# IntelRealSense/hand_tracking_samples

Measured on AMD Instinct MI355X. Metric: synthetic depth frames/sec (CNN+solver), 64x64x1 input, 17-bone hand, higher is better.
Workload: dtype f32; 1 GPU; BASELINE configs[2]: 1024 independent 64x64 frames per GPU, CNN + decode + 5-step MultiStepSim + 3 FitPointCloud passes (GJK + PGS), 17 bones; frames_per_gpu=1024, parallelism=single GPU

## Files before the change

### hand_tracking_samples_amd/csrc/ht_gjk.hip

```cpp
#include <stdlib.h>
#include <mutex>
#include "ht_device.hpp"
#include "ht_launch.hpp"

extern __shared__ __attribute__((aligned(16))) float4 g_sm[];

typedef float f32x2 __attribute__((ext_vector_type(2)));
struct support_t { int voff, n; v3 pos; v4 q; int outer; v3 opos; v4 oq; int sub, grp; };
struct mkpoint { v3 a, b; float t; __device__ __forceinline__ v3 p() const { return a - b; } };
struct simplex { v3 v; mkpoint W[4]; int count; };
struct gjk_hit { v3 normal, p0w, p1w; float separation; };

__device__ __forceinline__ v3 support_inner(const support_t &s, v3 dir)
{
	const v3 dl = qrot(qconj(s.q), dir);
	const float4 *vs = g_sm + s.voff;
	float4 q0 = vs[0];
	float best = dot(V3(q0.x, q0.y, q0.z), dl); int bi = 0;
	const f32x2 dlxy = { dl.x, dl.y };
	int i = 6 * s.sub;
	for (; i + 6 <= s.n; i += 6 * s.grp)
	{
		const float4 *g = vs + i;
		float d[6]; int id[6];
// ... 1056 lines not shown
		}
	}
}

size_t ht_contacts_workspace_bytes(int B) { (void)B; return 16; }

int ht_contacts_frames_per_block(const ht_model_dev &M, int B)
{
	const size_t fixed = (size_t)M.cvert_off[M.nb] * sizeof(float4) + sizeof(co_block) + (size_t)CO_OWN * 64 * 2 * (sizeof(co_req) + sizeof(int)) + CO_EPAQ * sizeof(co_job) + CO_NW * gjk_wave_stride();
	if (fixed + sizeof(co_frame) > 160 * 1024) return 0;
	int nfr = CO_MAXF;
	while (nfr > 1 && fixed + nfr * sizeof(co_frame) > 160 * 1024) nfr--;
	return B < nfr ? B : nfr;
}
#define CO_ORDER_SEG 4096
__global__ __launch_bounds__(1024) void k_contact_order(const int *__restrict__ work, int *__restrict__ order, int Ball, int nfr, int stride, unsigned slots, int epb)
{
	extern __shared__ int ko_w[];
	__shared__ int ko_ne;
	if (!((slots >> blockIdx.x) & 1u)) return;
	const int seg = (CO_ORDER_SEG / nfr) * nfr, f0 = blockIdx.y * seg, B = Ball - f0 < seg ? Ball - f0 : seg;
	const int blocks_all = (Ball + nfr - 1) / nfr, b0 = f0 / nfr;
	const int *w = work + (size_t)blockIdx.x * stride + f0;
	int *o = order + (size_t)blockIdx.x * stride;
	const int blocks = (B + nfr - 1) / nfr, B4 = (B + 3) & ~3;
	if (threadIdx.x == 0) ko_ne = 0;
	__syncthreads();
	int mine = 0;
	for (int i = threadIdx.x; i < B4; i += 1024)
	{
		const int v = i < B ? w[i] : -1;
		const int runs = v < 0 ? 0 : (v >> 16), pairs = v < 0 ? 0 : (v & 0xffff);
		ko_w[i] = v < 0 ? -1 : ((runs > 1023 ? 1023 : runs) << 20) | pairs;
		mine += runs > 0 ? 1 : 0;
	}
	if (mine) atomicAdd(&ko_ne, mine);
	for (int i = threadIdx.x; i < blocks * nfr; i += 1024) o[(i / blocks) * blocks_all + b0 + i % blocks] = Ball;
	__syncthreads();
	const int ne = ko_ne, ng = B - ne;
	if (epb > nfr) epb = nfr;
	if (epb * blocks < ne) epb = (ne + blocks - 1) / blocks;
	const int neb = (ne + epb - 1) / epb, ngb = blocks - neb;
	const int nfree = neb * nfr - ne;
	const int nheavy = ng - nfree > 0 ? ng - nfree : 0;
	for (int i = threadIdx.x; i < B; i += 1024)
	{
		const int wi = ko_w[i];
		int rank = 0;
		for (int j = 0; j < B4; j += 4)
		{
			const int4 k = *reinterpret_cast<const int4 *>(ko_w + j);
			rank += ((k.x > wi || (k.x == wi && j < i)) ? 1 : 0) + ((k.y > wi || (k.y == wi && j + 1 < i)) ? 1 : 0) + ((k.z > wi || (k.z == wi && j + 2 < i)) ? 1 : 0) + ((k.w > wi || (k.w == wi && j + 3 < i)) ? 1 : 0);
		}
		int nb_, base, r;
		if (rank < ne) { nb_ = neb; base = 0; r = rank; }
		else if (rank - ne < nheavy) { nb_ = ngb; base = neb; r = rank - ne; }
		else { nb_ = neb; base = 0; r = ne + (rank - ne - nheavy); }
		const int round = r / nb_, pos = r - round * nb_;
		o[round * blocks_all + b0 + base + ((round & 1) ? nb_ - 1 - pos : pos)] = f0 + i;
	}
}
void ht_launch_contact_order(const int *work, int *order, int B, int nfr, int stride, unsigned slots, int nslots, int epb, hipStream_t s)
{
	const int seg = (CO_ORDER_SEG / nfr) * nfr, nseg = (B + seg - 1) / seg;
	hipLaunchKernelGGL(k_contact_order, dim3(nslots, nseg), dim3(1024), (size_t)(((B < seg ? B : seg) + 3) & ~3) * sizeof(int), s, work, order, B, nfr, stride, slots, epb);
}
void ht_launch_contacts(const ht_model_dev &M, const float *state, float driftmax, float jiggle_sin, const int *active_flag, void *epa_ws, float *contacts, int *ncontacts, int B, hipStream_t s, bool beside_cloud_rows, int force_kernel, int few_frames,
                        const int *order, int *work_out)
{
	int *caps = reinterpret_cast<int *>(epa_ws);
	const int dbg = ht_tuning_flags();
	static bool attr_set[64];
	static std::mutex attr_lock;
	int dev = 0; (void)hipGetDevice(&dev); dev &= 63;
	std::unique_lock<std::mutex> lk(attr_lock);
	if (!attr_set[dev])
	{
		(void)hipFuncSetAttribute(reinterpret_cast<const void *>(k_contacts<1>), hipFuncAttributeMaxDynamicSharedMemorySize, 160 * 1024);
		(void)hipFuncSetAttribute(reinterpret_cast<const void *>(k_contacts<2>), hipFuncAttributeMaxDynamicSharedMemorySize, 160 * 1024);
		(void)hipFuncSetAttribute(reinterpret_cast<const void *>(k_contacts_coop), hipFuncAttributeMaxDynamicSharedMemorySize, 160 * 1024);
// ... 30 lines not shown
```

### hand_tracking_samples_amd/csrc/ht_host.hpp

```cpp
#pragma once
#include <map>
#include <string>
#include <vector>
#include "ht_device.hpp"

struct ht_comm_state;
struct ht_prof_entry { std::vector<hipEvent_t> ev; size_t used; float total_ms; int launches; };

struct ht_ctx
{
	bool ready = false, have_weights = false, profile = false;
	bool cnn_only = false;
	bool profile_phases = false;
	int B = 0, device = 0;
	int solver_build = 0;
	float *d_exact_lin = nullptr, *d_exact_ang = nullptr;
	int contact_kernel = 0;
	std::string err;
	hipStream_t stream = nullptr;
	hipStream_t last_user_stream = nullptr;
	hipStream_t side[2] = { nullptr, nullptr };
	hipEvent_t ev_fork = nullptr, ev_join[2] = { nullptr, nullptr }, ev_lap = nullptr;
	unsigned side_open = 0;
	hipEvent_t ev_job = nullptr, ev_seed = nullptr; bool job_pending = false; void *h_job_in = nullptr; size_t h_job_cap = 0;
// ... 22 lines not shown
	float *d_state[2] = { nullptr, nullptr };
	float *d_prev_err = nullptr; int *d_initializing = nullptr;
	float *d_err_old = nullptr, *d_err_new = nullptr; int *d_flags = nullptr, *d_nflags = nullptr;
	int *d_flist = nullptr, *d_nflist = nullptr;
	unsigned *d_nreset = nullptr; volatile unsigned *h_nreset = nullptr;
	unsigned nreset_seen[2] = { 0, 0 }; bool many_reset = false, tail_pending = false; int n_cu = 256;
	int last_reset_many = -1;
	float *d_rows = nullptr; int *d_nrows = nullptr;
	unsigned char *d_rowbody = nullptr;
	float *d_chamber = nullptr; int *d_nchamber = nullptr;
	float *d_tables = nullptr;
	float *d_chplanes = nullptr; int *d_chon = nullptr; bool planes_valid = false;
	int solve_tables = 0;
	int *d_accepted = nullptr;
	float *d_contacts = nullptr; int *d_ncontacts = nullptr;
	int *d_cwork = nullptr, *d_corder = nullptr;
	int *d_porder = nullptr;
	int *d_swork = nullptr, *d_sorder = nullptr; unsigned swork_mask = 0, sorder_mask = 0; int swork_B = 0;
	int cstride = 0, cwork_B = 0; unsigned cwork_mask = 0, corder_mask = 0;
	unsigned char *d_epa_ws = nullptr;
	float *d_scratch = nullptr;
	float *d_poses_out = nullptr, *d_start = nullptr;
	float *d_stage = nullptr;
	float *d_user_lin = nullptr; unsigned short *d_user_pos = nullptr; float *d_user_ang = nullptr; int *d_user_n = nullptr;
	int user_lin_cap = 0, user_ang_cap = 0;
	ht_comm_state *comm = nullptr;
	char *d_render = nullptr; size_t render_cap = 0;
	char *d_labels = nullptr; size_t labels_cap = 0;
	char *d_segment = nullptr; size_t segment_cap = 0;
	std::vector<float4> render_planes; std::vector<float> render_radii;
// ... 69 lines not shown
```

### hand_tracking_samples_amd/csrc/ht_solver.hip

```cpp
#include "ht_solve_shared.hpp"

template <int NGRP_, int NSUM_, int NANG_, int NIDX_, int AS_ = 2, int NCG_ = 0> struct lds_t
{
	static constexpr int NGRP = NGRP_, NSUM = NSUM_, NANG = NANG_, NIDX = NIDX_, MAXA2 = MAXA2_OF(AS_), NCG = NCG_;
	static constexpr int LIDLE = MAXG - 1;
	float pool[NGRP * LGRP] __attribute__((aligned(16)));
	float4 lin4[HT_MAXNB];
	float4 ang4[HT_MAXNB];
	float pos[HT_MAXNB][3], q[HT_MAXNB][4];
	float csum[NSUM];
	unsigned short cidx[NIDX > 0 ? NIDX : 2];
	float cg[NCG];
	int ccnt[HT_MAXNB], cstart[HT_MAXNB];
	signed char cextra[HT_MAXNB];
	union
	{
		unsigned lorder[MAXG];
		struct { unsigned short abody[128]; unsigned etmp[64]; } blk;
	};
	unsigned short lstart[MAXG + 2];
	unsigned aorder[MAXA2 + 1];
	unsigned short astart[MAXA2 + 2];
	int nlev_lin, nlev_ang, nray;
	union
// ... 1360 lines not shown
		if (bad) { pos = L3(bc + HT_BC_POS0); q = L4(bc + HT_BC_Q0); lin = V3(0, 0, 0); ang = V3(0, 0, 0); }
		if (a.zero_momenta) { lin = V3(0, 0, 0); ang = V3(0, 0, 0); }
		s[0] = pos.x; s[1] = pos.y; s[2] = pos.z; s[3] = q.x; s[4] = q.y; s[5] = q.z; s[6] = q.w;
		s[7] = lin.x; s[8] = lin.y; s[9] = lin.z; s[10] = ang.x; s[11] = ang.y; s[12] = ang.z;
		if (a.out_poses)
		{
			const v3 pu = apply(XF(pos, q), -L3(bc + HT_BC_COM));
			float *o = a.out_poses + ((size_t)b * nb + lane) * HT_POSE;
			o[0] = pu.x; o[1] = pu.y; o[2] = pu.z; o[3] = q.x; o[4] = q.y; o[5] = q.z; o[6] = q.w;
			if (lane == 0 && a.out_npts[b] < a.out_min_point_num) a.out_initializing[b] = 50;
		}
	}
	if (a.cost_out && lane == 0) a.cost_out[b] = (int)((clock64() - t_cost) >> 4);
}

__global__ __launch_bounds__(1024) void k_rank_desc(const int *__restrict__ work, int *__restrict__ order, int Ball, int stride, unsigned slots)
{
	__shared__ int rk_w[4096];
	if (!((slots >> blockIdx.x) & 1u)) return;
	const int f0 = blockIdx.y * 4096, B = Ball - f0 < 4096 ? Ball - f0 : 4096, B4 = (B + 3) & ~3;
	const int *w = work + (size_t)blockIdx.x * stride + f0;
	int *o = order + (size_t)blockIdx.x * stride + f0;
	for (int i = threadIdx.x; i < B4; i += 1024) rk_w[i] = i < B ? w[i] : -1;
	__syncthreads();
	for (int i = threadIdx.x; i < B; i += 1024)
	{
		const int wi = rk_w[i];
		int rank = 0;
		for (int j = 0; j < B4; j += 4)
		{
			const int4 k = *reinterpret_cast<const int4 *>(rk_w + j);
			rank += ((k.x > wi || (k.x == wi && j < i)) ? 1 : 0) + ((k.y > wi || (k.y == wi && j + 1 < i)) ? 1 : 0) + ((k.z > wi || (k.z == wi && j + 2 < i)) ? 1 : 0) + ((k.w > wi || (k.w == wi && j + 3 < i)) ? 1 : 0);
		}
		o[rank] = f0 + i;
	}
}
void ht_launch_rank_desc(const int *work, int *order, int B, int stride, unsigned slots, int nslots, hipStream_t s)
{
	hipLaunchKernelGGL(k_rank_desc, dim3(nslots, (B + 4095) / 4096), dim3(1024), 0, s, work, order, B, stride, slots);
}

#define SOLVE_ONLY_NCG 1440
static_assert(sizeof(lds_t<66, 1024, 126, 1024, 2, SOLVE_ONLY_NCG>) <= 40960, "the build for 1024 frames must fit four times into a CU's LDS");
static_assert(sizeof(lds_t<34, 584, 84, 0>) <= 20480, "the small build must leave room for eight frames per CU (160 KB of LDS)");
static_assert(HT_SCRATCH_TAIL * HT_CREC >= MAXG_CAP * LGRP + (MAXA_CAP_OF(4) + 4) * AROW + HT_CREC, "the tail of a frame's scratch slot must hold its linear groups, its angular records and the tuning record");
void ht_launch_solve(const ht_model_dev &M, const ht_physics_dev &ph, const solve_args &a, int B, hipStream_t s)
{
	const int pts = M.pts_bound > 0 ? M.pts_bound : M.pts_cap;
	const bool tile = M.nj + 8 + 1 <= 38 && pts <= 1024;
	int build = a.force_build;
	if (build == 7) { solve_args b = a; b.force_build = 0; b.two_body_levels = 1; ht_launch_solve(M, ph, b, B, s); return; }
	if (!build) build = tile ? (B <= 1024 && !a.shared_gpu ? 2 : 1) : 3;
	if (build >= 1 && build <= 3 && 13 + 6 * M.nj + a.ang_extra_bound > MAXA_CAP_OF(2)) build = 6;
	if (build == 2) hipLaunchKernelGGL((k_solve<66, 1024, 126, 1024, false, 2, SOLVE_ONLY_NCG>), dim3(B), dim3(64), 0, s, M, ph, a);
// ... 7 lines not shown
```

### hand_tracking_samples_amd/csrc/ht_solver_api.hip

```cpp
#include <string.h>
#include <stdlib.h>
#include "ht_device.hpp"
#include "ht_host.hpp"
#include "ht_launch.hpp"

#define CHECK_RANGE(ctx, first, n) do { if ((first) < 0 || (n) < 1 || (first) + (n) > (ctx)->B) { (ctx)->err = "slot range exceeds the capacity given to ht_create"; return HT_ERR_ARG; } } while (0)

static int scratch_stride(const ht_ctx *ctx) { return (int)ht_scratch_rows((size_t)ctx->model.pts_cap, (size_t)ctx->model.nb); }

static int dev_alloc_points(ht_ctx *ctx)
{
	const int r = dev_alloc(ctx, &ctx->d_ptsv, (size_t)ctx->B * ctx->model.pts_cap);
	return r || ctx->d_nptsv ? r : dev_alloc(ctx, &ctx->d_nptsv, (size_t)ctx->B);
}
static cloud_records cloud_rec(ht_ctx *ctx) { cloud_records r = { ctx->d_scratch, scratch_stride(ctx), ctx->d_rowbody, ctx->phys.deltaT }; return r; }
static bool exact_solver(const ht_ctx *ctx) { return ctx->solver_build == 5 || ctx->solver_build == 8; }
static const cloud_records *rec_or_rows(const ht_ctx *ctx, const cloud_records *cr) { return exact_solver(ctx) ? nullptr : cr; }
static void exact_args(ht_ctx *ctx, solve_args &a, bool cloud)
{
	a.force_build = exact_solver(ctx) ? 5 : ctx->solver_build;
	a.exact_lin = ctx->d_exact_lin; a.exact_ang = ctx->d_exact_ang;
	if (exact_solver(ctx) && cloud) { a.rows_cloud = ctx->d_rows; a.cloud_body = nullptr; }
}
#define REFUSE_EXACT_SOLVER(ctx) do { if (exact_solver(ctx)) { (ctx)->err = "the exact-order instantiation (ht_debug_solver_build 5) serves the update entry points only"; return HT_ERR_STATE; } } while (0)
// ... 4 lines not shown
	a.analysis = ctx->d_analysis; a.cams = ctx->d_cams; a.state = ctx->d_state[which]; a.scratch = ctx->d_scratch; a.scratch_stride = scratch_stride(ctx); a.batch = ctx->B;
	return a;
}
struct step_mix { bool angles, rays, cloud, chamber; float palm_drive; int arm_cone, zero_momenta; };
static step_mix mix_of_step(const ht_params &p, int st)
{
	const bool angles = (st < p.steps_keyangles) || p.angles_only, rays = (st < p.steps_keypoints) && !p.angles_only, cloud = (st >= p.steps_cloudstart) && !p.angles_only;
	step_mix m = { angles, rays, cloud, false, st < p.steps_palmangle ? 10000.0f : 0.0f, 1, 1 };
	return m;
}
static step_mix mix_of_pass() { step_mix m = { false, false, true, true, 0.0f, 0, 0 }; return m; }
static int step_slot(int st) { return st < 8 ? st : -1; }
static int pass_slot(int pass) { return pass >= 0 && pass < 8 ? 8 + pass : -1; }
static bool solve_history_on(const ht_ctx *ctx, int B) { return ctx->d_swork && B > ctx->n_cu * 8 && B + 8 <= ctx->cstride; }
struct solve_opts { const int *active = nullptr; int hist_slot = -1; bool tables = false, shared_gpu = false; float *poses_out = nullptr; const int *out_npts = nullptr; };
static void solve_step(ht_ctx *ctx, int which, const step_mix &m, int B, hipStream_t s, const solve_opts &o)
{
	solve_args a = solve_head(ctx, which, ctx->phys.use_collision != 0);
	a.rows_pre = m.chamber ? ctx->d_chamber : nullptr; a.n_pre = m.chamber ? ctx->d_nchamber : nullptr; a.pre_stride = 5 * ctx->model.nb;
	a.cloud_body = m.cloud ? ctx->d_rowbody : nullptr; a.n_cloud = ctx->d_nrows;
	a.active_flag = o.active; a.apply_angles = m.angles; a.drive_force = m.palm_drive; a.ray_rows = m.rays; a.arm_cone = m.arm_cone; a.zero_momenta = m.zero_momenta;
	a.steps_keyangles = ctx->par.steps_keyangles; a.min_cray_prob = ctx->par.min_cray_prob;
	a.dbg = ht_tuning_flags(); a.shared_gpu = o.shared_gpu ? 1 : 0; a.tables = o.tables ? ctx->d_tables : nullptr;
	exact_args(ctx, a, m.cloud);
	a.out_poses = o.poses_out; a.out_npts = o.out_npts; a.out_initializing = ctx->d_initializing; a.out_min_point_num = ctx->par.min_point_num;
	if (o.hist_slot >= 0 && o.hist_slot < HT_CONTACT_SLOTS && !o.active && !exact_solver(ctx) && solve_history_on(ctx, B) && B == ctx->swork_B)
	{
		a.cost_out = ctx->d_swork + (size_t)o.hist_slot * ctx->cstride;
		ctx->swork_mask |= 1u << o.hist_slot;
		if ((ctx->sorder_mask >> o.hist_slot) & 1u) a.frame_order = ctx->d_sorder + (size_t)o.hist_slot * ctx->cstride;
	}
	ht_launch_solve(ctx->model, ctx->phys, a, B, s);
}
static int solve_tables_mode(const ht_ctx *ctx)
{
	static const int env = ht_tuning_int("HT_TABLES", -1);
	const int m = env >= 0 ? env : ctx->solve_tables;
	return (m && ctx->d_tables && !exact_solver(ctx)) ? m : 0;
}
static bool solve_tables_on(const ht_ctx *ctx) { return solve_tables_mode(ctx) == 1; }
static void solve_prep(ht_ctx *ctx, int which, const step_mix &m, bool pose_only, const int *active, int B, hipStream_t s)
{
	prep_args a;
	memset(&a, 0, sizeof a);
	a.state = ctx->d_state[which]; a.analysis = ctx->d_analysis; a.cams = ctx->d_cams; a.active_flag = active;
	a.scratch = ctx->d_scratch; a.scratch_stride = scratch_stride(ctx); a.batch = ctx->B;
// ... 21 lines not shown
static inline void marks_dump() {}
#endif
struct contact_slot { const int *order; int *work; };
static contact_slot contact_history(ht_ctx *ctx, int slot, const int *active, int B)
{
	contact_slot c = { nullptr, nullptr };
	if (slot < 0 || slot >= HT_CONTACT_SLOTS || !ctx->d_cwork || active == ctx->d_flags || B != ctx->cwork_B) return c;
	c.work = ctx->d_cwork + (size_t)slot * ctx->cstride;
	ctx->cwork_mask |= 1u << slot;
	if ((ctx->corder_mask >> slot) & 1u) c.order = ctx->d_corder + (size_t)slot * ctx->cstride;
	return c;
}
static void launch_contacts(ht_ctx *ctx, int which, const int *active, int B, hipStream_t s, bool beside_cloud_rows = false, int slot = -1)
{
	const contact_slot ch = contact_history(ctx, slot, active, B);
	ht_launch_contacts(ctx->model, ctx->d_state[which], ctx->phys.driftmax, ctx->phys.jiggle_sin, active, ctx->d_epa_ws, ctx->d_contacts, ctx->d_ncontacts, B, s, beside_cloud_rows, ctx->contact_kernel,
	                   active && active == ctx->d_flags && !ctx->many_reset, ch.order, ch.work);
}
static void contact_orders(ht_ctx *ctx, int B, hipStream_t t)
{
	const int nfr = ht_contacts_frames_per_block(ctx->model, B);
	ctx->corder_mask = 0;
	if (ctx->d_cwork && ctx->cwork_B == B && ctx->cwork_mask && nfr > 1 && B + 8 <= ctx->cstride && ctx->contact_kernel != 2)
	{
		static const int epb_env = ht_tuning_int("HT_CONTACT_EPB", 0);
		const int blocks = (B + nfr - 1) / nfr;
		ht_launch_contact_order(ctx->d_cwork, ctx->d_corder, B, nfr, ctx->cstride, ctx->cwork_mask, HT_CONTACT_SLOTS, epb_env > 0 ? epb_env : blocks > ctx->n_cu ? nfr : 1, t);
		ctx->corder_mask = ctx->cwork_mask;
	}
	ctx->cwork_mask = 0; ctx->cwork_B = B;
	ctx->sorder_mask = 0;
	if (solve_history_on(ctx, B) && ctx->swork_B == B && ctx->swork_mask)
	{
		ht_launch_rank_desc(ctx->d_swork, ctx->d_sorder, B, ctx->cstride, ctx->swork_mask, HT_CONTACT_SLOTS, t);
		ctx->sorder_mask = ctx->swork_mask;
	}
	ctx->swork_mask = 0; ctx->swork_B = B;
}
static void fork(ht_ctx *ctx, hipStream_t s) { (void)hipEventRecord(ctx->ev_fork, s); for (int i = 0; i < 2; i++) (void)hipStreamWaitEvent(ctx->side[i], ctx->ev_fork, 0); ctx->side_open |= 3u; }
static void fork1(ht_ctx *ctx, hipStream_t s, int i) { (void)hipEventRecord(ctx->ev_fork, s); (void)hipStreamWaitEvent(ctx->side[i], ctx->ev_fork, 0); ctx->side_open |= 1u << i; }
static void join1(ht_ctx *ctx, hipStream_t s, int i) { (void)hipEventRecord(ctx->ev_join[i], ctx->side[i]); (void)hipStreamWaitEvent(s, ctx->ev_join[i], 0); ctx->side_open &= ~(1u << i); }
static void join(ht_ctx *ctx, hipStream_t s, int n) { for (int i = 0; i < n; i++) join1(ctx, s, i); }
static void join_open(ht_ctx *ctx, hipStream_t s) { for (int i = 0; i < 2; i++) if ((ctx->side_open >> i) & 1u) join1(ctx, s, i); }

struct steps_on
{
	hipStream_t s; int from = 0, to = 1 << 30; const int *active = nullptr; int side = 0; bool prof = true, shared_gpu = false, rows = true, solve = true;
	explicit steps_on(hipStream_t stream) : s(stream) {}
	steps_on &steps(int first, int end = 1 << 30) { from = first; to = end; return *this; }
	steps_on &frames(const int *flags) { active = flags; return *this; }
	steps_on &all_frames() { active = nullptr; return *this; }
	steps_on &rows_beside(int i) { side = i; return *this; }
	steps_on &in_order() { side = -1; return *this; }
	steps_on &unprofiled() { prof = false; return *this; }
	steps_on &shares_gpu() { shared_gpu = true; return *this; }
	steps_on &rows_only() { solve = false; return *this; }
// ... 123 lines not shown
static void update_planes(ht_ctx *ctx, const update_call &u, hipStream_t t)
{
	const ht_params &p = ctx->par;
	if (u.mode == UPD_CNN_MODEL || u.mode == UPD_KICKSTART || p.angles_only || p.mainthreadpasses < 1) return;
	ht_launch_chamber_planes(ctx->model, p.subsample_voxel ? ctx->d_ptsv : ctx->d_pts, p.subsample_voxel ? ctx->d_nptsv : ctx->d_npts, p.min_point_num, p.boundary_planes, ctx->d_chplanes, ctx->d_chon, u.B, t); ctx->planes_valid = true;
}
static void update_fit_error_old(ht_ctx *ctx, const update_call &u, hipStream_t t)
{
	const ht_params &p = ctx->par;
	ht_fit_after dec; memset(&dec, 0, sizeof dec);
	dec.mode = 1; dec.reset_thr = p.full_reset_on_error; dec.angles_only = p.angles_only; dec.flags = ctx->d_flags; dec.nflags = ctx->d_nflags; dec.list = ctx->d_flist; dec.nlist = ctx->d_nflist; dec.nreset = ctx->d_nreset;
	ht_launch_fit_error(ctx->model, ctx->d_state[0], ctx->d_pts, ctx->d_npts, u.d_depth, u.img_cams, u.iw, u.ih, p.bone_sum_error_scale, ctx->d_err_old, u.B, t, &dec);
}
static void update_beside_net(ht_ctx *ctx, const update_call &u)
{
	hipStream_t t = ctx->side[1];
	fork(ctx, u.s);
	update_planes(ctx, u, t);
	contact_orders(ctx, u.B, t);
	if (u.mode == UPD_FULL && !(u.d_start && !u.fs)) ht_launch_set_pose(ctx->d_state[1], ctx->d_state[0], ctx->model.nb, u.B, 2, t);
	update_fit_error_old(ctx, u, t);
}
static void update_net(ht_ctx *ctx, const update_call &u, bool overlap)
{
	const frame_src *fs = u.fs; const bool direct = fs && fs->direct; hipStream_t s = u.s;
	ht_prof_scope ps(ctx, direct ? "cnn128" : "cnn", s, true);
	if (direct) ht_launch_cnn(ctx->cnnw128, ctx->d_in128, ctx->d_act1_128, ctx->d_act2_128, ctx->d_act3, ctx->d_logits, u.B, s, fs->direct, overlap);
	else ht_launch_cnn(ctx->cnnw, ctx->d_cnn_in, ctx->d_act1, ctx->d_act2, ctx->d_act3, ctx->d_logits, u.B, s, 64, overlap);
	ht_launch_softmax_decode(ctx->d_logits, u.d_cnn_out ? u.d_cnn_out : ctx->d_cnn_out, ctx->d_cams, ctx->d_analysis, 1, u.B, s, direct ? fs->direct / 16 : 4);
}
static void resets_short(ht_ctx *ctx, int B, hipStream_t s)
{
	reset_path(ctx, true, ctx->par.steps_unibody, B, ctx->side[0], s, ctx->many_reset);
	multistep(ctx, B, steps_on(s).steps(0, 1).frames(ctx->d_nflags).rows_beside(0).shares_gpu());
	join(ctx, s, 1); reset_tail(ctx);
	multistep(ctx, B, steps_on(s).steps(0, 1).frames(ctx->d_flags).rows_beside(0));
// ... 7 lines not shown
	join(ctx, s, 1); reset_tail(ctx);
	multistep(ctx, B, steps_on(s).steps(join_step).all_frames().rows_beside(0));
}
static void resets_lap(ht_ctx *ctx, int B, hipStream_t s)
{
	hipStream_t u = ctx->side[0];
	const int *reset_frames = ctx->d_flags, *batch_frames = ctx->d_nflags;
	mark("fork", s);
	reset_path(ctx, true, ctx->par.steps_unibody, B, s, s, ctx->many_reset); mark("reset kernel done", s);
	multistep(ctx, B, steps_on(u).steps(0, 1).frames(batch_frames).in_order().unprofiled().shares_gpu()); mark("batch step 0 done", u);
	multistep(ctx, B, steps_on(s).steps(0, 1).frames(reset_frames).in_order().rows_only()); mark("reset frames contacts done", s);
	(void)hipEventRecord(ctx->ev_lap, s); (void)hipStreamWaitEvent(u, ctx->ev_lap, 0);
	multistep(ctx, B, steps_on(s).steps(0, 1).frames(reset_frames).in_order().solve_only()); mark("reset frames step 0 done", s);
	multistep(ctx, B, steps_on(u).steps(1, 2).frames(batch_frames).in_order().unprofiled().rows_only()); mark("batch step 1 rows done", u);
	multistep(ctx, B, steps_on(s).steps(1, 2).frames(reset_frames).rows_beside(1).rows_only()); mark("reset frames step 1 rows done", s);
	join(ctx, s, 1); reset_tail(ctx);
	multistep(ctx, B, steps_on(s).steps(1, 2).all_frames().solve_only()); mark("step 1 done", s);
	multistep(ctx, B, steps_on(s).steps(2).all_frames().rows_beside(0)); mark("MultiStepSim done", s);
}
static void update_resets(ht_ctx *ctx, const update_call &u)
{
	hipStream_t s = u.s; join1(ctx, s, 1);
	static const int join_step = ht_tuning_int("HT_RESET_JOIN", 0);
	fork(ctx, s);
	const unsigned frames = ctx->h_nreset[0], updates = ctx->h_nreset[1];
	if (updates != ctx->nreset_seen[1])
	{
		ctx->many_reset = (frames - ctx->nreset_seen[0]) / (updates - ctx->nreset_seen[1]) > (unsigned)ctx->n_cu;
		ctx->nreset_seen[0] = frames; ctx->nreset_seen[1] = updates;
	}
	static const bool no_lap = ht_tuning_env("HT_NO_STEP1_LAP");
	if (join_step > 0) resets_joined_late(ctx, u.B, s, join_step);
	else if (ctx->par.steps >= 2 && !no_lap) resets_lap(ctx, u.B, s);
	else resets_short(ctx, u.B, s);
}
static void update_accept(ht_ctx *ctx, const update_call &u)
{
	const ht_params &p = ctx->par;
	ht_fit_after acc; memset(&acc, 0, sizeof acc);
	acc.mode = 2; acc.hand = u.mode == UPD_CNN_MODEL ? nullptr : ctx->d_state[0]; acc.other = ctx->d_state[1]; acc.err_old = ctx->d_err_old; acc.prev_err = ctx->d_prev_err;
	acc.initializing = ctx->d_initializing; acc.accepted = ctx->d_accepted; acc.nb = ctx->model.nb; acc.min_point_num = p.min_point_num; acc.always_take_cnn = p.always_take_cnn;
	acc.angles_only = p.angles_only; acc.accum_thr = p.accum_error_threshold; ht_prof_scope ps(ctx, "fit_error", u.s, true);
	ht_launch_fit_error(ctx->model, ctx->d_state[1], ctx->d_pts, ctx->d_npts, u.d_depth, u.img_cams, u.iw, u.ih, p.bone_sum_error_scale, ctx->d_err_new, u.B, u.s, &acc);
}
static void update_passes(ht_ctx *ctx, const update_call &u)
{
	const ht_params &p = ctx->par;
	const int passes = p.angles_only ? 0 : p.mainthreadpasses;
// ... 434 lines not shown
}
extern "C" int ht_debug_reset_flags(ht_ctx *ctx, int *flags, int n)
{
	if (!ctx || !flags || n < 0 || n > ctx->B) return HT_ERR_ARG;
	ht_device_guard dev_guard_(ctx->device);
	HIPCHK(ctx, hipStreamSynchronize(ctx->stream));
	HIPCHK(ctx, hipMemcpy(flags, ctx->d_flags, (size_t)n * sizeof(int), hipMemcpyDeviceToHost));
	return HT_OK;
}
extern "C" int ht_debug_contact_kernel(ht_ctx *ctx, int which)
{
	if (!ctx || which < 0 || which > 2) return HT_ERR_ARG;
	ctx->contact_kernel = which;
	return HT_OK;
}
extern "C" int ht_debug_solve_tables(ht_ctx *ctx, int on)
{
	if (!ctx || !ctx->ready) return HT_ERR_ARG;
	ht_device_guard dev_guard_(ctx->device);
	if (on < 0 || on > 2) return HT_ERR_ARG;
	if (on) { const int r = ht_alloc_solve_tables(ctx); if (r) return r; }
	ctx->solve_tables = on;
	return HT_OK;
}
extern "C" int ht_debug_solve_tables_header(ht_ctx *ctx, int B, int *hdr)
{
	if (!ctx || !ctx->ready || !hdr || B < 1 || B > ctx->B || !ctx->d_tables) return HT_ERR_ARG;
	ht_device_guard dev_guard_(ctx->device);
	if (ht_sync_all(ctx) != hipSuccess) return HT_ERR_HIP;
	if (hipMemcpy2D(hdr, 32 * sizeof(int), ctx->d_tables, (size_t)TB_WORDS * sizeof(float), 32 * sizeof(int), B, hipMemcpyDeviceToHost) != hipSuccess) return HT_ERR_HIP;
// ... 233 lines not shown
```

### hand_tracking_samples_amd/native.py

```python
import ctypes as C
import os

import numpy as np

from . import build as _build

HERE = os.path.dirname(os.path.abspath(__file__))
HT_OK = 0
CNN_IN, CNN_OUT, CNNB_COUNT, POSE, STATE, CAM, ANALYSIS = 4096, 2304, 9458400, 7, 13, 12, 84
MAXPTS, ROW, CONTACT = 4096, 16, 12
LABELS_SEGMENT_FRAME = 1
TRAIN_ACT = (("a1", 57600, (16, 60, 60)), ("a3", 3600, (16, 15, 15)), ("a5", 9216, (64, 12, 12)), ("a6", 2304, (2304,)), ("a8", 2048, (2048,)))
TRAIN_ERR = (("e9", 2304, (2304,)), ("e7", 2048, (2048,)), ("e6", 2304, (2304,)), ("part3", 57600, (16, 3600)), ("sqp", 9, (9,)), (None, 7, None))

SYMBOLS = (
    "ht_create", "ht_destroy", "ht_model_bake", "ht_last_error", "ht_get_params", "ht_set_params", "ht_model_info", "ht_config_read", "ht_scale",
    "ht_cnn_load_weights", "ht_cnn_eval", "ht_cnn_eval_dev", "ht_cnn_load_weights_sized", "ht_cnn_eval_sized", "ht_cnn_eval_sized_dev", "ht_cnn_train", "ht_cnn_get_weights", "ht_expected_cnn", "ht_expected_cnn_full",
    "ht_expected_cnn_batch", "ht_expected_cnn_dev", "ht_cnn_input_dev", "ht_cnn_train_dev", "ht_cnn_train_batch_dev", "ht_cnn_train_batch", "ht_debug_train_batch_buffers",
    "ht_model_open", "ht_model_close", "ht_model_error", "ht_model_counts", "ht_model_body", "ht_model_body_mesh", "ht_model_body_sdmesh", "ht_model_hitcheck", "ht_model_hitcheck_mesh", "ht_model_render_mesh", "ht_model_scale", "ht_render_mesh_depth", "ht_render_mesh_depth_dev",
    "ht_tracker_reset", "ht_get_state", "ht_set_state", "ht_get_tracker_flags", "ht_set_tracker_flags", "ht_update_sync", "ht_update_dev", "ht_update_frames_sync", "ht_update_frames_dev", "ht_update_direct_sync", "ht_update_direct_dev", "ht_update_cnn_model_sync", "ht_get_cnn_results", "ht_get_cnn_layers", "ht_frames_overflow", "ht_reserve_points", "ht_point_capacity", "ht_capacity_events", "ht_segment_vr", "ht_segment_vr_dev", "ht_render_depth", "ht_render_depth_dev", "ht_slowfit", "ht_set_points", "ht_fit_rows", "ht_physics_update",
    "ht_stage_prepare", "ht_stage_decode", "ht_stage_fit_error", "ht_stage_cloud_rows", "ht_stage_contacts", "ht_stage_fit",
    "ht_stage_multistep", "ht_stage_multistep_range", "ht_stage_scratch_unibody", "ht_stage_chamber", "ht_profile_enable", "ht_profile_read", "ht_debug_solve_stats", "ht_debug_contact_stats", "ht_debug_solver_build", "ht_debug_reset_flags", "ht_debug_reset_organisation", "ht_update_passes_sync", "ht_job_start", "ht_job_poll", "ht_job_wait", "ht_job_collect", "ht_debug_contact_kernel", "ht_contact_capacity", "ht_debug_solve_tables", "ht_debug_solve_tables_header", "ht_debug_train_buffers",
    "ht_comm_available", "ht_comm_unique_id", "ht_comm_init", "ht_comm_info", "ht_gather_poses_dev", "ht_gather_wait", "ht_gather_wait_host", "ht_comm_destroy",
)


class Params(C.Structure):
    _fields_ = [("full_reset_on_error", C.c_float), ("angles_only", C.c_int), ("always_take_cnn", C.c_int), ("drangey", C.c_float), ("boundary_planes", C.c_int),
                ("microforce", C.c_float), ("cloudforce_max_point", C.c_float), ("cloudforce_max_sum", C.c_float), ("mainthreadpasses", C.c_int),
                ("subsample_fraction", C.c_int), ("min_point_num", C.c_int), ("accum_error_threshold", C.c_float), ("min_cray_prob", C.c_float),
                ("steps", C.c_int), ("steps_keypoints", C.c_int), ("steps_keyangles", C.c_int), ("steps_palmangle", C.c_int), ("steps_cloudstart", C.c_int), ("steps_unibody", C.c_int),
                ("physics_iterations", C.c_int), ("physics_iterations_post", C.c_int), ("physics_use_collision", C.c_int),
                ("physics_weak_force", C.c_float), ("bone_sum_error_scale", C.c_float), ("unibody_force", C.c_float),
                ("subsample_voxel", C.c_int), ("subsample_size", C.c_float)]


class HTError(RuntimeError):
# ... 76 lines not shown
    L.ht_segment_vr.argtypes = [vp, C.POINTER(C.c_uint16), fp, C.c_int, C.c_int, C.c_int, C.c_int, C.c_float, C.c_float, C.c_float, C.POINTER(C.c_uint16), fp]
    L.ht_segment_vr_dev.argtypes = [vp, vp, vp, C.c_int, C.c_int, C.c_int, C.c_int, C.c_float, C.c_float, C.c_float, vp, vp, vp]
    L.ht_render_depth.argtypes = [vp, fp, fp, C.c_int, C.c_int, C.c_float, C.c_int, u16p, C.POINTER(C.c_int8)]
    L.ht_render_depth_dev.argtypes = [vp, vp, vp, C.c_int, C.c_int, C.c_float, C.c_int, vp, vp, vp]
    L.ht_render_mesh_depth.argtypes = [vp, fp, fp, C.c_int, C.c_int, C.c_float, C.c_float, C.c_int, u16p, C.POINTER(C.c_int8)]
    L.ht_render_mesh_depth_dev.argtypes = [vp, vp, vp, C.c_int, C.c_int, C.c_float, C.c_float, C.c_int, vp, vp, vp]
    L.ht_model_hitcheck_mesh.argtypes = [vp, fp, fp, fp, fp, fp, ip, ip]
    L.ht_model_render_mesh.argtypes = [vp, fp, fp, C.c_int, C.c_int, C.c_float, C.c_float, u16p, C.POINTER(C.c_int8)]
    L.ht_model_scale.argtypes = [vp, C.c_float]
    L.ht_profile_read.argtypes = [vp, C.c_int, C.c_int, C.c_char_p, C.c_int, fp, ip, ip]
    L.ht_debug_solve_stats.argtypes = [vp, C.c_int, fp, C.c_int]
    L.ht_debug_solver_build.argtypes = [vp, C.c_int]
    L.ht_debug_reset_organisation.argtypes = [vp, ip]
    L.ht_debug_reset_flags.argtypes = [vp, ip, C.c_int]
    L.ht_debug_contact_kernel.argtypes = [vp, C.c_int]
    L.ht_debug_solve_tables.argtypes = [vp, C.c_int]
    L.ht_contact_capacity.argtypes = [vp, ip, ip, ip, ip]
    L.ht_debug_solve_tables_header.argtypes = [vp, C.c_int, ip]
    L.ht_comm_unique_id.argtypes = [vp]
    L.ht_comm_init.argtypes = [vp, C.c_int, C.c_int, vp]
    L.ht_comm_info.argtypes = [vp, ip, ip]
    L.ht_gather_poses_dev.argtypes = [vp, vp, vp, C.c_int, C.c_int, vp]
    L.ht_gather_wait.argtypes = [vp, C.c_int, vp]
    L.ht_gather_wait_host.argtypes = [vp, C.c_int]
    L.ht_comm_available.argtypes = []
    L.ht_comm_destroy.argtypes = [vp]
    L.ht_debug_contact_stats.argtypes = [vp, C.c_int, fp, C.c_int]
    for name in SYMBOLS:
        if name not in ("ht_last_error", "ht_model_error"):
            getattr(L, name).restype = C.c_int
# ... 302 lines not shown

    def gather_wait_host(self, slot):
        self._chk(self.L.ht_gather_wait_host(self.h, int(slot)))

    def debug_reset_flags(self, n):
        f = np.zeros(n, np.int32)
        self._chk(self.L.ht_debug_reset_flags(self.h, f.ctypes.data_as(C.POINTER(C.c_int)), n))
        return f

    def debug_solver_build(self, which):
        self._chk(self.L.ht_debug_solver_build(self.h, int(which)))

    def debug_contact_kernel(self, which):
        self._chk(self.L.ht_debug_contact_kernel(self.h, int(which)))

    def contact_capacity(self):
        v = [C.c_int() for _ in range(4)]
        self._chk(self.L.ht_contact_capacity(self.h, *[C.byref(x) for x in v]))
        return tuple(x.value for x in v)

    def debug_solve_tables(self, on):
        self._chk(self.L.ht_debug_solve_tables(self.h, int(on)))

    def debug_solve_tables_header(self, B):
        h = np.zeros((B, 32), np.int32)
        self._chk(self.L.ht_debug_solve_tables_header(self.h, B, _i(h)))
        return h

    def debug_contact_stats(self, B, reset=True):
        out = np.zeros((B, 24), np.float32)
# ... 175 lines not shown
```

### include/ht_mi355x.h

```cpp
#ifndef HT_MI355X_H
#define HT_MI355X_H
#include <stddef.h>
#include <stdint.h>

#ifdef __cplusplus
extern "C" {
#endif

#define HT_OK 0
#define HT_ERR_ARG 1
#define HT_ERR_IO 2
#define HT_ERR_HIP 3
#define HT_ERR_STATE 4

#define HT_CNN_IN 4096
#define HT_CNN_OUT 2304
#define HT_CNNB_COUNT 9458400
#define HT_CNN128_IN 16384
#define HT_CNNB128_COUNT 30429920
#define HT_POSE 7
#define HT_STATE 13
#define HT_CAM 12
#define HT_MAX_POINTS 4096
#define HT_POINTS_LIMIT 76800
// ... 130 lines not shown
int ht_comm_unique_id(void *id128);
int ht_comm_init(ht_ctx *ctx, int world, int rank, const void *id128);
int ht_comm_info(ht_ctx *ctx, int *world, int *rank);
int ht_gather_poses_dev(ht_ctx *ctx, const float *d_local, float *d_all, int frames, int slot, void *stream);
int ht_gather_wait(ht_ctx *ctx, int slot, void *stream);
int ht_comm_destroy(ht_ctx *ctx);

int ht_profile_enable(ht_ctx *ctx, int on);
int ht_profile_read(ht_ctx *ctx, int reset, int max_entries, char *names, int name_stride, float *total_ms, int *launches, int *n_entries);
int ht_debug_solve_stats(ht_ctx *ctx, int B, float *out, int reset);
int ht_debug_contact_stats(ht_ctx *ctx, int B, float *out, int reset);
int ht_debug_solver_build(ht_ctx *ctx, int which);
int ht_debug_reset_flags(ht_ctx *ctx, int *flags, int n);
int ht_debug_reset_organisation(ht_ctx *ctx, int *many);
int ht_debug_contact_kernel(ht_ctx *ctx, int which);
int ht_debug_solve_tables(ht_ctx *ctx, int mode);
int ht_debug_train_buffers(ht_ctx *ctx, float *act, size_t n_act, float *err, size_t n_err);
int ht_debug_solve_tables_header(ht_ctx *ctx, int B, int *hdr);

#ifdef __cplusplus
}
#endif
#endif
```

Measured before the change: 235,100 frames/s.

## Split order/rank kernels across blocks and reschedule side-stream update branches

The ranking kernels (k_rank_desc, k_contact_order) now spread each frame's O(B) rank count across a third grid dimension of 256-thread blocks, instead of one 1024-thread block looping over all frames. Each block redundantly loads the shared work array. The contact-order fill of empty slots is now computed per place rather than written up front. In update_beside_net, fit-error work goes to side stream 1 and the orders/planes to side stream 0, with a tuning-only check that table readers have joined side 0. The reset path also delays joining side 0 when the step-1 overlap is used, which is meant to shorten the critical path, at the cost of ordering risk between streams.

```diff
diff --git a/hand_tracking_samples_amd/csrc/ht_gjk.hip b/hand_tracking_samples_amd/csrc/ht_gjk.hip
--- a/hand_tracking_samples_amd/csrc/ht_gjk.hip
+++ b/hand_tracking_samples_amd/csrc/ht_gjk.hip
@@ -1094,20 +1094,22 @@
 	return B < nfr ? B : nfr;
 }
 #define CO_ORDER_SEG 4096
-__global__ __launch_bounds__(1024) void k_contact_order(const int *__restrict__ work, int *__restrict__ order, int Ball, int nfr, int stride, unsigned slots, int epb)
+#define CO_ORDER_PART 256
+__global__ __launch_bounds__(CO_ORDER_PART) void k_contact_order(const int *__restrict__ work, int *__restrict__ order, int Ball, int nfr, int stride, unsigned slots, int epb)
 {
 	extern __shared__ int ko_w[];
 	__shared__ int ko_ne;
 	if (!((slots >> blockIdx.x) & 1u)) return;
 	const int seg = (CO_ORDER_SEG / nfr) * nfr, f0 = blockIdx.y * seg, B = Ball - f0 < seg ? Ball - f0 : seg;
 	const int blocks_all = (Ball + nfr - 1) / nfr, b0 = f0 / nfr;
+	const int blocks = (B + nfr - 1) / nfr, B4 = (B + 3) & ~3, places = blocks * nfr;
+	if ((int)blockIdx.z * CO_ORDER_PART >= places) return;
 	const int *w = work + (size_t)blockIdx.x * stride + f0;
 	int *o = order + (size_t)blockIdx.x * stride;
-	const int blocks = (B + nfr - 1) / nfr, B4 = (B + 3) & ~3;
 	if (threadIdx.x == 0) ko_ne = 0;
 	__syncthreads();
 	int mine = 0;
-	for (int i = threadIdx.x; i < B4; i += 1024)
+	for (int i = threadIdx.x; i < B4; i += CO_ORDER_PART)
 	{
 		const int v = i < B ? w[i] : -1;
 		const int runs = v < 0 ? 0 : (v >> 16), pairs = v < 0 ? 0 : (v & 0xffff);
@@ -1115,7 +1117,6 @@
 		mine += runs > 0 ? 1 : 0;
 	}
 	if (mine) atomicAdd(&ko_ne, mine);
-	for (int i = threadIdx.x; i < blocks * nfr; i += 1024) o[(i / blocks) * blocks_all + b0 + i % blocks] = Ball;
 	__syncthreads();
 	const int ne = ko_ne, ng = B - ne;
 	if (epb > nfr) epb = nfr;
@@ -1123,27 +1124,33 @@
 	const int neb = (ne + epb - 1) / epb, ngb = blocks - neb;
 	const int nfree = neb * nfr - ne;
 	const int nheavy = ng - nfree > 0 ? ng - nfree : 0;
-	for (int i = threadIdx.x; i < B; i += 1024)
-	{
-		const int wi = ko_w[i];
-		int rank = 0;
-		for (int j = 0; j < B4; j += 4)
-		{
-			const int4 k = *reinterpret_cast<const int4 *>(ko_w + j);
-			rank += ((k.x > wi || (k.x == wi && j < i)) ? 1 : 0) + ((k.y > wi || (k.y == wi && j + 1 < i)) ? 1 : 0) + ((k.z > wi || (k.z == wi && j + 2 < i)) ? 1 : 0) + ((k.w > wi || (k.w == wi && j + 3 < i)) ? 1 : 0);
-		}
-		int nb_, base, r;
-		if (rank < ne) { nb_ = neb; base = 0; r = rank; }
-		else if (rank - ne < nheavy) { nb_ = ngb; base = neb; r = rank - ne; }
-		else { nb_ = neb; base = 0; r = ne + (rank - ne - nheavy); }
-		const int round = r / nb_, pos = r - round * nb_;
-		o[round * blocks_all + b0 + base + ((round & 1) ? nb_ - 1 - pos : pos)] = f0 + i;
-	}
+	const int i = blockIdx.z * CO_ORDER_PART + threadIdx.x;
+	if (i < places)
+	{
+		const int round = i / blocks, col = i - round * blocks;
+		const bool first = col < neb;
+		const int nb_ = first ? neb : ngb, p = first ? col : col - neb, count = first ? ne + (ng - nheavy) : nheavy;
+		if (round * nb_ + ((round & 1) ? nb_ - 1 - p : p) >= count) o[round * blocks_all + b0 + col] = Ball;
+	}
+	if (i >= B) return;
+	const int wi = ko_w[i];
+	int rank = 0;
+	for (int j = 0; j < B4; j += 4)
+	{
+		const int4 k = *reinterpret_cast<const int4 *>(ko_w + j);
+		rank += ((k.x > wi || (k.x == wi && j < i)) ? 1 : 0) + ((k.y > wi || (k.y == wi && j + 1 < i)) ? 1 : 0) + ((k.z > wi || (k.z == wi && j + 2 < i)) ? 1 : 0) + ((k.w > wi || (k.w == wi && j + 3 < i)) ? 1 : 0);
+	}
+	int nb_, base, r;
+	if (rank < ne) { nb_ = neb; base = 0; r = rank; }
+	else if (rank - ne < nheavy) { nb_ = ngb; base = neb; r = rank - ne; }
+	else { nb_ = neb; base = 0; r = ne + (rank - ne - nheavy); }
+	const int round = r / nb_, pos = r - round * nb_;
+	o[round * blocks_all + b0 + base + ((round & 1) ? nb_ - 1 - pos : pos)] = f0 + i;
 }
 void ht_launch_contact_order(const int *work, int *order, int B, int nfr, int stride, unsigned slots, int nslots, int epb, hipStream_t s)
 {
-	const int seg = (CO_ORDER_SEG / nfr) * nfr, nseg = (B + seg - 1) / seg;
-	hipLaunchKernelGGL(k_contact_order, dim3(nslots, nseg), dim3(1024), (size_t)(((B < seg ? B : seg) + 3) & ~3) * sizeof(int), s, work, order, B, nfr, stride, slots, epb);
+	const int seg = (CO_ORDER_SEG / nfr) * nfr, nseg = (B + seg - 1) / seg, first = B < seg ? B : seg, places = (first + nfr - 1) / nfr * nfr;
+	hipLaunchKernelGGL(k_contact_order, dim3(nslots, nseg, (places + CO_ORDER_PART - 1) / CO_ORDER_PART), dim3(CO_ORDER_PART), (size_t)((first + 3) & ~3) * sizeof(int), s, work, order, B, nfr, stride, slots, epb);
 }
 void ht_launch_contacts(const ht_model_dev &M, const float *state, float driftmax, float jiggle_sin, const int *active_flag, void *epa_ws, float *contacts, int *ncontacts, int B, hipStream_t s, bool beside_cloud_rows, int force_kernel, int few_frames,
                         const int *order, int *work_out)
diff --git a/hand_tracking_samples_amd/csrc/ht_host.hpp b/hand_tracking_samples_amd/csrc/ht_host.hpp
--- a/hand_tracking_samples_amd/csrc/ht_host.hpp
+++ b/hand_tracking_samples_amd/csrc/ht_host.hpp
@@ -60,6 +60,7 @@
 	int solve_tables = 0;
 	int *d_accepted = nullptr;
 	float *d_contacts = nullptr; int *d_ncontacts = nullptr;
+	bool tables_out = false;
 	int *d_cwork = nullptr, *d_corder = nullptr;
 	int *d_porder = nullptr;
 	int *d_swork = nullptr, *d_sorder = nullptr; unsigned swork_mask = 0, sorder_mask = 0; int swork_B = 0;
diff --git a/hand_tracking_samples_amd/csrc/ht_solver.hip b/hand_tracking_samples_amd/csrc/ht_solver.hip
--- a/hand_tracking_samples_amd/csrc/ht_solver.hip
+++ b/hand_tracking_samples_amd/csrc/ht_solver.hip
@@ -1398,30 +1398,32 @@
 	if (a.cost_out && lane == 0) a.cost_out[b] = (int)((clock64() - t_cost) >> 4);
 }
 
-__global__ __launch_bounds__(1024) void k_rank_desc(const int *__restrict__ work, int *__restrict__ order, int Ball, int stride, unsigned slots)
+#define RANK_PART 256
+__global__ __launch_bounds__(RANK_PART) void k_rank_desc(const int *__restrict__ work, int *__restrict__ order, int Ball, int stride, unsigned slots)
 {
 	__shared__ int rk_w[4096];
 	if (!((slots >> blockIdx.x) & 1u)) return;
 	const int f0 = blockIdx.y * 4096, B = Ball - f0 < 4096 ? Ball - f0 : 4096, B4 = (B + 3) & ~3;
+	if ((int)blockIdx.z * RANK_PART >= B) return;
 	const int *w = work + (size_t)blockIdx.x * stride + f0;
 	int *o = order + (size_t)blockIdx.x * stride + f0;
-	for (int i = threadIdx.x; i < B4; i += 1024) rk_w[i] = i < B ? w[i] : -1;
+	for (int i = threadIdx.x; i < B4; i += RANK_PART) rk_w[i] = i < B ? w[i] : -1;
 	__syncthreads();
-	for (int i = threadIdx.x; i < B; i += 1024)
-	{
-		const int wi = rk_w[i];
-		int rank = 0;
-		for (int j = 0; j < B4; j += 4)
-		{
-			const int4 k = *reinterpret_cast<const int4 *>(rk_w + j);
-			rank += ((k.x > wi || (k.x == wi && j < i)) ? 1 : 0) + ((k.y > wi || (k.y == wi && j + 1 < i)) ? 1 : 0) + ((k.z > wi || (k.z == wi && j + 2 < i)) ? 1 : 0) + ((k.w > wi || (k.w == wi && j + 3 < i)) ? 1 : 0);
-		}
-		o[rank] = f0 + i;
-	}
+	const int i = blockIdx.z * RANK_PART + threadIdx.x;
+	if (i >= B) return;
+	const int wi = rk_w[i];
+	int rank = 0;
+	for (int j = 0; j < B4; j += 4)
+	{
+		const int4 k = *reinterpret_cast<const int4 *>(rk_w + j);
+		rank += ((k.x > wi || (k.x == wi && j < i)) ? 1 : 0) + ((k.y > wi || (k.y == wi && j + 1 < i)) ? 1 : 0) + ((k.z > wi || (k.z == wi && j + 2 < i)) ? 1 : 0) + ((k.w > wi || (k.w == wi && j + 3 < i)) ? 1 : 0);
+	}
+	o[rank] = f0 + i;
 }
 void ht_launch_rank_desc(const int *work, int *order, int B, int stride, unsigned slots, int nslots, hipStream_t s)
 {
-	hipLaunchKernelGGL(k_rank_desc, dim3(nslots, (B + 4095) / 4096), dim3(1024), 0, s, work, order, B, stride, slots);
+	const int seg = B < 4096 ? B : 4096;
+	hipLaunchKernelGGL(k_rank_desc, dim3(nslots, (B + 4095) / 4096, (seg + RANK_PART - 1) / RANK_PART), dim3(RANK_PART), 0, s, work, order, B, stride, slots);
 }
 
 #define SOLVE_ONLY_NCG 1440
diff --git a/hand_tracking_samples_amd/csrc/ht_solver_api.hip b/hand_tracking_samples_amd/csrc/ht_solver_api.hip
--- a/hand_tracking_samples_amd/csrc/ht_solver_api.hip
+++ b/hand_tracking_samples_amd/csrc/ht_solver_api.hip
@@ -42,6 +42,12 @@
 static int pass_slot(int pass) { return pass >= 0 && pass < 8 ? 8 + pass : -1; }
 static bool solve_history_on(const ht_ctx *ctx, int B) { return ctx->d_swork && B > ctx->n_cu * 8 && B + 8 <= ctx->cstride; }
 struct solve_opts { const int *active = nullptr; int hist_slot = -1; bool tables = false, shared_gpu = false; float *poses_out = nullptr; const int *out_npts = nullptr; };
+static void table_read_on(const ht_ctx *ctx, hipStream_t s)
+{
+#ifdef HT_TUNING
+	if (ctx->tables_out && s != ctx->side[0]) { fprintf(stderr, "a launch table read on a stream that has not joined side stream 0\n"); abort(); }
+#endif
+}
 static void solve_step(ht_ctx *ctx, int which, const step_mix &m, int B, hipStream_t s, const solve_opts &o)
 {
 	solve_args a = solve_head(ctx, which, ctx->phys.use_collision != 0);
@@ -58,6 +64,7 @@
 		ctx->swork_mask |= 1u << o.hist_slot;
 		if ((ctx->sorder_mask >> o.hist_slot) & 1u) a.frame_order = ctx->d_sorder + (size_t)o.hist_slot * ctx->cstride;
 	}
+	if (a.frame_order) table_read_on(ctx, s);
 	ht_launch_solve(ctx->model, ctx->phys, a, B, s);
 }
 static int solve_tables_mode(const ht_ctx *ctx)
@@ -109,6 +116,7 @@
 static void launch_contacts(ht_ctx *ctx, int which, const int *active, int B, hipStream_t s, bool beside_cloud_rows = false, int slot = -1)
 {
 	const contact_slot ch = contact_history(ctx, slot, active, B);
+	if (ch.order) table_read_on(ctx, s);
 	ht_launch_contacts(ctx->model, ctx->d_state[which], ctx->phys.driftmax, ctx->phys.jiggle_sin, active, ctx->d_epa_ws, ctx->d_contacts, ctx->d_ncontacts, B, s, beside_cloud_rows, ctx->contact_kernel,
 	                   active && active == ctx->d_flags && !ctx->many_reset, ch.order, ch.work);
 }
@@ -134,7 +142,7 @@
 }
 static void fork(ht_ctx *ctx, hipStream_t s) { (void)hipEventRecord(ctx->ev_fork, s); for (int i = 0; i < 2; i++) (void)hipStreamWaitEvent(ctx->side[i], ctx->ev_fork, 0); ctx->side_open |= 3u; }
 static void fork1(ht_ctx *ctx, hipStream_t s, int i) { (void)hipEventRecord(ctx->ev_fork, s); (void)hipStreamWaitEvent(ctx->side[i], ctx->ev_fork, 0); ctx->side_open |= 1u << i; }
-static void join1(ht_ctx *ctx, hipStream_t s, int i) { (void)hipEventRecord(ctx->ev_join[i], ctx->side[i]); (void)hipStreamWaitEvent(s, ctx->ev_join[i], 0); ctx->side_open &= ~(1u << i); }
+static void join1(ht_ctx *ctx, hipStream_t s, int i) { (void)hipEventRecord(ctx->ev_join[i], ctx->side[i]); (void)hipStreamWaitEvent(s, ctx->ev_join[i], 0); ctx->side_open &= ~(1u << i); if (i == 0) ctx->tables_out = false; }
 static void join(ht_ctx *ctx, hipStream_t s, int n) { for (int i = 0; i < n; i++) join1(ctx, s, i); }
 static void join_open(ht_ctx *ctx, hipStream_t s) { for (int i = 0; i < 2; i++) if ((ctx->side_open >> i) & 1u) join1(ctx, s, i); }
 
@@ -288,12 +296,14 @@
 }
 static void update_beside_net(ht_ctx *ctx, const update_call &u)
 {
-	hipStream_t t = ctx->side[1];
+	hipStream_t fit = ctx->side[1], rest = ctx->side[0];
+	mark("update start", u.s);
 	fork(ctx, u.s);
-	update_planes(ctx, u, t);
-	contact_orders(ctx, u.B, t);
-	if (u.mode == UPD_FULL && !(u.d_start && !u.fs)) ht_launch_set_pose(ctx->d_state[1], ctx->d_state[0], ctx->model.nb, u.B, 2, t);
-	update_fit_error_old(ctx, u, t);
+	if (u.mode == UPD_FULL && !(u.d_start && !u.fs)) ht_launch_set_pose(ctx->d_state[1], ctx->d_state[0], ctx->model.nb, u.B, 2, fit);
+	update_fit_error_old(ctx, u, fit); mark("carried FitError done", fit);
+	contact_orders(ctx, u.B, rest); mark("orders done", rest);
+	update_planes(ctx, u, rest); mark("planes done", rest);
+	ctx->tables_out = true;
 }
 static void update_net(ht_ctx *ctx, const update_call &u, bool overlap)
 {
@@ -331,14 +341,19 @@
 	multistep(ctx, B, steps_on(s).steps(0, 1).frames(reset_frames).in_order().solve_only()); mark("reset frames step 0 done", s);
 	multistep(ctx, B, steps_on(u).steps(1, 2).frames(batch_frames).in_order().unprofiled().rows_only()); mark("batch step 1 rows done", u);
 	multistep(ctx, B, steps_on(s).steps(1, 2).frames(reset_frames).rows_beside(1).rows_only()); mark("reset frames step 1 rows done", s);
-	join(ctx, s, 1); reset_tail(ctx);
+	join(ctx, s, 1); mark("side branch back", s); reset_tail(ctx);
 	multistep(ctx, B, steps_on(s).steps(1, 2).all_frames().solve_only()); mark("step 1 done", s);
 	multistep(ctx, B, steps_on(s).steps(2).all_frames().rows_beside(0)); mark("MultiStepSim done", s);
 }
 static void update_resets(ht_ctx *ctx, const update_call &u)
 {
-	hipStream_t s = u.s; join1(ctx, s, 1);
+	hipStream_t s = u.s; mark("net done", s);
 	static const int join_step = ht_tuning_int("HT_RESET_JOIN", 0);
+	static const bool no_lap = ht_tuning_env("HT_NO_STEP1_LAP");
+	const bool lap = join_step <= 0 && ctx->par.steps >= 2 && !no_lap;
+	join1(ctx, s, 1);
+	if (!lap) join1(ctx, s, 0);
+	mark(lap ? "reset decision back" : "side branch back", s);
 	fork(ctx, s);
 	const unsigned frames = ctx->h_nreset[0], updates = ctx->h_nreset[1];
 	if (updates != ctx->nreset_seen[1])
@@ -346,9 +361,8 @@
 		ctx->many_reset = (frames - ctx->nreset_seen[0]) / (updates - ctx->nreset_seen[1]) > (unsigned)ctx->n_cu;
 		ctx->nreset_seen[0] = frames; ctx->nreset_seen[1] = updates;
 	}
-	static const bool no_lap = ht_tuning_env("HT_NO_STEP1_LAP");
 	if (join_step > 0) resets_joined_late(ctx, u.B, s, join_step);
-	else if (ctx->par.steps >= 2 && !no_lap) resets_lap(ctx, u.B, s);
+	else if (lap) resets_lap(ctx, u.B, s);
 	else resets_short(ctx, u.B, s);
 }
 static void update_accept(ht_ctx *ctx, const update_call &u)
@@ -813,6 +827,33 @@
 	ctx->contact_kernel = which;
 	return HT_OK;
 }
+template <class F> static int debug_order_table(ht_ctx *ctx, const int *work, int B, int n_out, int *order_out, F launch)
+{
+	const int stride = B + 8;
+	int *d = nullptr;
+	HIPCHK(ctx, hipMalloc(&d, (size_t)2 * stride * sizeof(int)));
+	hipStream_t s = ctx->stream;
+	hipError_t e = hipMemcpyAsync(d, work, (size_t)B * sizeof(int), hipMemcpyHostToDevice, s);
+	if (e == hipSuccess) e = hipMemsetAsync(d + stride, 0xff, (size_t)stride * sizeof(int), s);
+	if (e == hipSuccess) { launch(d, d + stride, stride, s); e = hipGetLastError(); }
+	if (e == hipSuccess) e = hipMemcpyAsync(order_out, d + stride, (size_t)n_out * sizeof(int), hipMemcpyDeviceToHost, s);
+	if (e == hipSuccess) e = hipStreamSynchronize(s); else (void)hipStreamSynchronize(s);
+	(void)hipFree(d);
+	HIPCHK(ctx, e);
+	return HT_OK;
+}
+extern "C" int ht_debug_contact_order(ht_ctx *ctx, const int *work, int B, int nfr, int epb, int *order_out)
+{
+	CHECK_READY(ctx);
+	if (!work || !order_out || B < 1 || nfr < 1 || nfr > 8 || epb < 1) return HT_ERR_ARG;
+	return debug_order_table(ctx, work, B, (B + nfr - 1) / nfr * nfr, order_out, [&](const int *w, int *o, int stride, hipStream_t s) { ht_launch_contact_order(w, o, B, nfr, stride, 1u, 1, epb, s); });
+}
+extern "C" int ht_debug_rank_desc(ht_ctx *ctx, const int *work, int B, int *order_out)
+{
+	CHECK_READY(ctx);
+	if (!work || !order_out || B < 1) return HT_ERR_ARG;
+	return debug_order_table(ctx, work, B, B, order_out, [&](const int *w, int *o, int stride, hipStream_t s) { ht_launch_rank_desc(w, o, B, stride, 1u, 1, s); });
+}
 extern "C" int ht_debug_solve_tables(ht_ctx *ctx, int on)
 {
 	if (!ctx || !ctx->ready) return HT_ERR_ARG;
diff --git a/hand_tracking_samples_amd/native.py b/hand_tracking_samples_amd/native.py
--- a/hand_tracking_samples_amd/native.py
+++ b/hand_tracking_samples_amd/native.py
@@ -20,7 +20,7 @@
     "ht_model_open", "ht_model_close", "ht_model_error", "ht_model_counts", "ht_model_body", "ht_model_body_mesh", "ht_model_body_sdmesh", "ht_model_hitcheck", "ht_model_hitcheck_mesh", "ht_model_render_mesh", "ht_model_scale", "ht_render_mesh_depth", "ht_render_mesh_depth_dev",
     "ht_tracker_reset", "ht_get_state", "ht_set_state", "ht_get_tracker_flags", "ht_set_tracker_flags", "ht_update_sync", "ht_update_dev", "ht_update_frames_sync", "ht_update_frames_dev", "ht_update_direct_sync", "ht_update_direct_dev", "ht_update_cnn_model_sync", "ht_get_cnn_results", "ht_get_cnn_layers", "ht_frames_overflow", "ht_reserve_points", "ht_point_capacity", "ht_capacity_events", "ht_segment_vr", "ht_segment_vr_dev", "ht_render_depth", "ht_render_depth_dev", "ht_slowfit", "ht_set_points", "ht_fit_rows", "ht_physics_update",
     "ht_stage_prepare", "ht_stage_decode", "ht_stage_fit_error", "ht_stage_cloud_rows", "ht_stage_contacts", "ht_stage_fit",
-    "ht_stage_multistep", "ht_stage_multistep_range", "ht_stage_scratch_unibody", "ht_stage_chamber", "ht_profile_enable", "ht_profile_read", "ht_debug_solve_stats", "ht_debug_contact_stats", "ht_debug_solver_build", "ht_debug_reset_flags", "ht_debug_reset_organisation", "ht_update_passes_sync", "ht_job_start", "ht_job_poll", "ht_job_wait", "ht_job_collect", "ht_debug_contact_kernel", "ht_contact_capacity", "ht_debug_solve_tables", "ht_debug_solve_tables_header", "ht_debug_train_buffers",
+    "ht_stage_multistep", "ht_stage_multistep_range", "ht_stage_scratch_unibody", "ht_stage_chamber", "ht_profile_enable", "ht_profile_read", "ht_debug_solve_stats", "ht_debug_contact_stats", "ht_debug_solver_build", "ht_debug_reset_flags", "ht_debug_reset_organisation", "ht_update_passes_sync", "ht_job_start", "ht_job_poll", "ht_job_wait", "ht_job_collect", "ht_debug_contact_kernel", "ht_debug_contact_order", "ht_debug_rank_desc", "ht_contact_capacity", "ht_debug_solve_tables", "ht_debug_solve_tables_header", "ht_debug_train_buffers",
     "ht_comm_available", "ht_comm_unique_id", "ht_comm_init", "ht_comm_info", "ht_gather_poses_dev", "ht_gather_wait", "ht_gather_wait_host", "ht_comm_destroy",
 )
 
@@ -127,6 +127,8 @@
     L.ht_debug_reset_organisation.argtypes = [vp, ip]
     L.ht_debug_reset_flags.argtypes = [vp, ip, C.c_int]
     L.ht_debug_contact_kernel.argtypes = [vp, C.c_int]
+    L.ht_debug_contact_order.argtypes = [vp, ip, C.c_int, C.c_int, C.c_int, ip]
+    L.ht_debug_rank_desc.argtypes = [vp, ip, C.c_int, ip]
     L.ht_debug_solve_tables.argtypes = [vp, C.c_int]
     L.ht_contact_capacity.argtypes = [vp, ip, ip, ip, ip]
     L.ht_debug_solve_tables_header.argtypes = [vp, C.c_int, ip]
@@ -459,6 +461,17 @@
     def debug_contact_kernel(self, which):
         self._chk(self.L.ht_debug_contact_kernel(self.h, int(which)))
 
+    def debug_contact_order(self, work, nfr, epb):
+        work = _c(work, np.int32); B = len(work); blocks = (B + nfr - 1) // nfr
+        out = np.empty(blocks * nfr, np.int32)
+        self._chk(self.L.ht_debug_contact_order(self.h, _i(work), B, int(nfr), int(epb), _i(out)))
+        return out.reshape(nfr, blocks)
+
+    def debug_rank_desc(self, work):
+        work = _c(work, np.int32); out = np.empty(len(work), np.int32)
+        self._chk(self.L.ht_debug_rank_desc(self.h, _i(work), len(work), _i(out)))
+        return out
+
     def contact_capacity(self):
         v = [C.c_int() for _ in range(4)]
         self._chk(self.L.ht_contact_capacity(self.h, *[C.byref(x) for x in v]))
diff --git a/include/ht_mi355x.h b/include/ht_mi355x.h
--- a/include/ht_mi355x.h
+++ b/include/ht_mi355x.h
@@ -168,6 +168,8 @@
 int ht_debug_reset_flags(ht_ctx *ctx, int *flags, int n);
 int ht_debug_reset_organisation(ht_ctx *ctx, int *many);
 int ht_debug_contact_kernel(ht_ctx *ctx, int which);
+int ht_debug_contact_order(ht_ctx *ctx, const int *work, int B, int nfr, int epb, int *order_out);
+int ht_debug_rank_desc(ht_ctx *ctx, const int *work, int B, int *order_out);
 int ht_debug_solve_tables(ht_ctx *ctx, int mode);
 int ht_debug_train_buffers(ht_ctx *ctx, float *act, size_t n_act, float *err, size_t n_err);
 int ht_debug_solve_tables_header(ht_ctx *ctx, int B, int *hdr);
```

Result: faster. 237,600 frames/s (median of 6 runs) (+1.0%).
